# fjall-rs/lsm-tree

Measured on AMD Instinct MI355X. Metric: device-resident data-block decode+encode GiB/s, 1 M × 4 KiB blocks, higher is better.
Workload: dtype u8; 1 GPU; BASELINE configs[1]/[2]: encode + decode round trip of 1 M x 4 KiB data blocks, device-resident; blocks_per_gpu=1048576, items_per_gpu=54525952, block_bytes_per_gpu=3953267212, restart_interval=16, key_len=16, val_len=64, parallelism=shard1 (independent block batches, no collective)

## Files before the change

### lsm-tree_amd/csrc/encode.hip

```cpp
#include <hip/hip_runtime.h>

#include <math.h>

#include <algorithm>
#include <cstddef>
#include <type_traits>

#include "block_format.hpp"
#include "decode.hpp"
#include "encode.hpp"
#include "scan.hpp"
#include "fill.hpp"

namespace lsmgpu {

constexpr uint32_t kPlanHuge = 1, kPlanBad = 2, kPlanMedium = 4, kPlanBig = 8;
constexpr uint32_t kPlanHugeGpu = 16;
constexpr uint32_t kImgMedium = 20 * 1024;
constexpr uint32_t kImgBig = 96 * 1024;
constexpr uint32_t kListBigWaves = 8;
constexpr uint32_t kE3HashChunk = 4096;
constexpr uint64_t kListedOne = 1ULL << 40, kOffMask = kListedOne - 1;

struct alignas(16) BlockPlan {
// ... 1058 lines not shown
      for (uint32_t q = 0; q < kPW; ++q) {
        if (!ok[q]) continue;
        const uint32_t n = bst[jq[q] + 1] - bst[jq[q]];
        const uint32_t buckets = bucket_count(n, P.ratio);
        const uint32_t hw = (buckets > 0 && (n + ri - 1) / ri <= kHashMaxPointers) ? buckets : 0;
        uint32_t hb = kNoBucket;
        if (hw && hw < kNeedHash) {
          if (m[q].klen <= 16)
            hb = (uint32_t)(xxh3_64_le16(m[q].klen, WinReader8{wb[q].lo, wb[q].hi},
                                         WinReader64{wb[q].lo, wb[q].hi}) % hw);
          else
            hb = kNeedHash, P.hb_fix[0] = 1;
        }
        P.hbucket[(uint64_t)base + t0 + q] = (uint16_t)hb;
      }
    }
    wave_lds_sync();
    uint32_t nq[kPW];
    uint64_t hq[kPW];
#pragma unroll
    for (uint32_t q = 0; q < kPW; ++q) {
      nq[q] = 0;
      hq[q] = 0;
      wa[q] = wb[q];
      if (ok[q] && jjq[q] % ri != 0) {
        const uint32_t h = base + t0 + q - jjq[q] % ri;
        const bool in = h >= base;
        const uint64_t hko = in ? (uint64_t)wkos[h - base] : hk_ko;
        const uint32_t hkl = in ? wkls[h - base] : hk_kl;
        nq[q] = min(hkl, m[q].klen);
        hq[q] = hko;
        wa[q] = in ? wkwin[h - base] : hk_win;
      }
    }
#pragma unroll
    for (uint32_t q = 0; q < kPW; ++q) {
      if (!nq[q]) continue;
      const uint64_t x0 = wa[q].lo ^ wb[q].lo, x1 = wa[q].hi ^ wb[q].hi;
      const uint32_t n = nq[q];
      uint32_t sh;
      if (x0) sh = min(n, (uint32_t)(__builtin_ctzll(x0) >> 3));
      else if (x1) sh = min(n, 8 + (uint32_t)(__builtin_ctzll(x1) >> 3));
      else sh = n <= 16 ? n : lcp_tail(P.it.keys, hq[q], m[q].ko, n);
      m[q].sh = sh;
    }
    uint64_t rec[kPW], tsum = 0;
#pragma unroll
    for (uint32_t q = 0; q < kPW; ++q) {
      rec[q] = ok[q] ? item_record_len(P, m[q], jjq[q] % ri == 0) : 0;
      tsum += rec[q];
    }
    const uint64_t incl = wave_incl_scan_u64(tsum);
    uint64_t ex = carry + incl - tsum;
    uint64_t exq[kPW];
#pragma unroll
    for (uint32_t q = 0; q < kPW; ++q) {
      exq[q] = ex;
      if (ok[q]) {
        const uint32_t jb = jq[q], jj = jjq[q], ridx = jj / ri;
        const uint32_t n = bst[jb + 1] - bst[jb];
        if (jj == 0) bfirst[jb] = ex;
        if (jj + 1 == n) bend[jb] = ex + rec[q];
        if (jj == ridx * ri && ridx == (n - 1) / ri) lhead[jb] = ex;
      }
      ex += rec[q];
    }
    wave_lds_sync();
#pragma unroll
    for (uint32_t q = 0; q < kPW; ++q) {
      if (ok[q]) {
        const uint32_t jj = jjq[q], ridx = jj / ri;
        const bool head = jj == ridx * ri;
        const uint64_t roff = exq[q] - bfirst[jq[q]];
        const uint32_t x = head ? ridx : m[q].sh;
        P.erec[(uint64_t)base + t0 + q] =
            bst[jq[q] + 1] - bst[jq[q]] > kGItems
                ? (uint32_t)min(roff, (uint64_t)0xFFFFFFFFu)
                : (uint32_t)min(roff, (uint64_t)0x7FFF) | (head ? kErecHead : 0u) | (min(x, 0xFFFFu) << 16);
      }
    }
    carry += wave_bcast_u64(incl, kWave - 1);
    {
      const uint32_t last = min(ie, base + kPWStep) - 1, ll = (last - base) / kPW, lq = (last - base) % kPW;
      uint32_t jsel = jjq[0];
#pragma unroll
      for (uint32_t q = 1; q < kPW; ++q) jsel = lq == q ? jjq[q] : jsel;
      const uint32_t jjl = __builtin_amdgcn_readlane((int)jsel, (int)ll);
      const uint32_t h = last - jjl % ri;
      if (h >= base) {
        hk_ko = wkos[h - base];
        hk_kl = wkls[h - base];
        hk_win = wkwin[h - base];
      }
    }
    wave_lds_sync();
  }
  __syncthreads();
  if (tid >= nb) return;
  const uint32_t b = b0 + tid, s = bst[tid], e = bst[tid + 1];
  bool bad = !mono || e <= s || badf[tid] || start_past_items(P, b + 1);
  const uint32_t n = bad ? 0 : e - s;
  const uint64_t recs = bad ? 0 : bend[tid] - bfirst[tid], last_head = bad ? 0 : lhead[tid] - bfirst[tid];
  const uint32_t bin_len = n ? (n + ri - 1) / ri : 0;
  const uint32_t step = last_head <= 0xFFFF ? 2 : 4;
  const uint32_t buckets = bucket_count(n, P.ratio);
  const uint32_t hash_w = (buckets > 0 && bin_len <= kHashMaxPointers) ? buckets : 0;
  const uint64_t total = kHdrLen + recs + 1 + (uint64_t)bin_len * step + hash_w + kTrailerLen;
  if (recs > 0xFFFFFFF0ULL || total > 0xFFFFFF00ULL) bad = true;
  const uint64_t ks = koff<kOW>(P, s), ke = koff<kOW>(P, e);
  const uint64_t vs = voff<kOW>(P, s), ve = voff<kOW>(P, e);
  uint32_t flags = 0;
  if (bad) {
    flags = kPlanBad;
    P.status[b] = ST_BAD_ARG;
  } else if (!group_fits(n, ke - ks, ve - vs, total, hash_w)) {
    const uint64_t need = e2_need(total, hash_w);
    flags = need <= kImgMedium ? kPlanMedium : need <= kImgBig ? kPlanBig : kPlanHuge;
  }
  const BlockPlan pl{(uint32_t)recs, bin_len, hash_w, step | (flags << 8)};
  const uint64_t size = (bad ? 0 : total) | ((flags & (kPlanMedium | kPlanBig | kPlanHuge)) ? kListedOne : 0);
  P.plans[b] = pl;
  if (kFused) {
    fplan[tid] = pl;
    fsize[tid] = size;
    if (size & ~kOffMask) P.status[b] = ST_INCOMPLETE;
  } else {
    P.sizes[b] = size;
  }
  P.kspan[b] = ks;
  P.vspan[b] = vs;
  if (b + 1 == P.n_blocks) {
    P.kspan[b + 1] = ke;
    P.vspan[b + 1] = ve;
  }
}

template <bool kBkt, int kOW>
__global__ __launch_bounds__(256) __attribute__((amdgpu_waves_per_eu(4))) void encode_plan_wave_kernel(EncodeParams P) {
  __shared__ PlanWaveLds S;
  const uint32_t b0 = blockIdx.x * P.plan_bpw;
  plan_wave_run<kBkt, kOW, false>(P, b0, min(P.plan_bpw, P.n_blocks - b0), S, nullptr, nullptr);
}

struct GBlk {
  uint32_t it0, n;
  uint32_t img, plen;
  uint32_t recs, bin_len;
  uint32_t step, hash_w;
  uint32_t hash_base, u0;
  uint32_t nbk, spare;
};
static_assert(sizeof(GBlk) == 48, "GBlk");

struct GroupLds {
  uint8_t keys[kGKeys + kGSlack];
  uint8_t vals[kGVals + kGSlack];
  uint8_t img[kGImg + kGSlack];
  uint32_t uni[kGUnion / 4];
  GBlk blk[2][kGBlocks];
  LongSecret secret;
};
static_assert(offsetof(GroupLds, uni) - offsetof(GroupLds, vals) >= sizeof(PlanWaveLds), "plan LDS over the stage");
static_assert(offsetof(GroupLds, vals) % 16 == 0, "plan LDS alignment");
static_assert(kGRunFused * (sizeof(BlockPlan) + 8) + 16 <= kGUnion, "fused plan outputs in uni");


__device__ __forceinline__ void lds_copy(uint8_t* dst, uint32_t d, const uint8_t* src, uint32_t s, uint32_t n,
                                         uint32_t rot, uint32_t done = 0) {
  if (!n) return;
  const uint32_t h = min(n, (4u - (d & 3u)) & 3u);
  uint32_t hb[3];
#pragma unroll
  for (uint32_t k = 0; k < 3; ++k)
    if (k < h) hb[k] = src[s + k];
#pragma unroll
  for (uint32_t k = 0; k < 3; ++k)
    if (k < h) dst[d + k] = (uint8_t)hb[k];
  if (n == h) return;
  const uint32_t d1 = d + h + 4 * done, e = d + n, body = ((e & ~3u) - d1) >> 2;
  const uint32_t sp = s + h + 4 * done, sh = sp & 3u;
  const uint32_t* s32 = reinterpret_cast<const uint32_t*>(src + (sp & ~3u));
  uint32_t* d32 = reinterpret_cast<uint32_t*>(dst + d1);
  uint32_t q = ((rot & 31u) * body) >> 5;
  constexpr uint32_t U = 4;
  const uint32_t w0 = body ? s32[0] : 0;
  uint32_t carry = body ? s32[q] : 0;
  for (uint32_t j0 = 0; j0 < body; j0 += U) {
    uint32_t hi[U], at[U];
#pragma unroll
    for (uint32_t t = 0; t < U; ++t) {
      uint32_t p = q + t;
      p = p >= body ? p - body : p;
      at[t] = p;
      if (j0 + t < body) hi[t] = s32[p + 1];
    }
#pragma unroll
    for (uint32_t t = 0; t < U; ++t) {
      if (j0 + t < body) {
        const uint32_t lo = t == 0 ? carry : (at[t] == 0 ? w0 : hi[t - 1]);
        d32[at[t]] = alignbyte(hi[t], lo, sh);
      }
    }
    q += U;
    q = q >= body ? q - body : q;
    carry = q == 0 ? w0 : hi[U - 1];
  }
  const uint32_t t0 = d1 + 4 * body;
  uint32_t tb[3];
#pragma unroll
  for (uint32_t k = 0; k < 3; ++k)
    if (t0 + k < e) tb[k] = src[s + (t0 + k - d)];
#pragma unroll
  for (uint32_t k = 0; k < 3; ++k)
    if (t0 + k < e) dst[t0 + k] = (uint8_t)tb[k];
}

#ifdef LSM_NO_UNIFORM_COPY
constexpr bool kUniformCopy = false;
#else
constexpr bool kUniformCopy = true;
#endif
constexpr uint32_t kUniformMin = 4;
__device__ __forceinline__ uint32_t lds_copy_uniform(uint8_t* dst, uint32_t d, const uint8_t* src, uint32_t s,
                                                     uint32_t n, bool has, uint32_t rot) {
  if (!kUniformCopy) return 0;
  const uint32_t h = min(n, (4u - (d & 3u)) & 3u);
  const uint32_t body = n > h ? (((d + n) & ~3u) - (d + h)) >> 2 : 0u;
  const uint32_t B = wave_min_u32(has ? body : 0xFFFFFFFFu);
  if (B < kUniformMin || B == 0xFFFFFFFFu) return 0;
  if (has) {
    const uint8_t* sb = src + ((s + h) & ~3u);
    uint8_t* db = dst + d + h;
    const uint32_t sh = (s + h) & 3u, B4 = 4 * B;
    auto ld = [&](uint32_t x) { return *reinterpret_cast<const uint32_t*>(sb + x); };
    auto st = [&](uint32_t x, uint32_t v) { *reinterpret_cast<uint32_t*>(db + x) = v; };
    constexpr uint32_t U = kUniformMin;
    uint32_t x = (((rot & 31u) * B) >> 5) * 4;
    const uint32_t w0 = ld(0);
    uint32_t carry = ld(x);
    for (uint32_t j = 0; j < B; j += U) {
      uint32_t at[U], hi[U];
#pragma unroll
      for (uint32_t t = 0; t < U; ++t) {
        const uint32_t y = x + 4 * t;
        at[t] = t == 0 ? x : min(y, y - B4);
        hi[t] = ld(at[t] + 4);
      }
#pragma unroll
      for (uint32_t t = 0; t < U; ++t) {
        const uint32_t lo = at[t] == 0 ? w0 : (t == 0 ? carry : hi[t - 1]);
        st(at[t], alignbyte(hi[t], lo, sh));
      }
      carry = hi[U - 1];
      x += 4 * U;
      x = min(x, x - B4);
    }
    if (body > B) {
      st(B4, alignbyte(ld(B4 + 4), ld(B4), sh));
      return B + 1;
    }
  }
  return B;
}

__device__ __forceinline__ uint32_t lds_put_leb(uint8_t* dst, uint32_t pos, uint64_t v) {
  while (v >= 0x80) {
    dst[pos++] = (uint8_t)(v | 0x80);
    v >>= 7;
  }
  dst[pos++] = (uint8_t)v;
  return pos;
}

__device__ __forceinline__ void group_barrier() {
  __builtin_amdgcn_fence(__ATOMIC_RELEASE, "workgroup", "local");
  __builtin_amdgcn_s_barrier();
  __builtin_amdgcn_fence(__ATOMIC_ACQUIRE, "workgroup", "local");
}

__device__ __forceinline__ void group_barrier_lds() {
  asm volatile("s_waitcnt lgkmcnt(0)\n\ts_barrier" ::: "memory");
}

#ifdef LSM_DIAG
#define ENC_PHASE(i)                                 \
  if (P.diag & 0x80) {                              \
    const uint64_t t_ = __builtin_amdgcn_s_memtime(); \
    ph_acc[i] += (uint32_t)(t_ - t_last);            \
    t_last = t_;                                     \
  }
#else
#define ENC_PHASE(i)
#endif

__device__ __forceinline__ uint32_t block_of_item(const EncodeParams& P, uint32_t i) {
  uint32_t lo = 0, hi = P.n_blocks;
  while (hi - lo > 1) {
    const uint32_t mid = (lo + hi) >> 1;
    if (clamped_start(P, mid) <= i) lo = mid;
    else hi = mid;
  }
  return lo;
}

constexpr uint64_t kE1pBad = 1ULL << 63;
constexpr uint32_t kE1pMaxBpw = 4;
__device__ __forceinline__ uint64_t e1p_add(uint64_t a, uint64_t b) {
  return ((a | b) & kE1pBad) | ((a + b) & ~kE1pBad);
}

__device__ __forceinline__ uint64_t shfl_down64(uint64_t v, int o) {
  return (uint64_t)(uint32_t)__shfl_down((int)(uint32_t)v, o) |
         ((uint64_t)(uint32_t)__shfl_down((int)(uint32_t)(v >> 32), o) << 32);
}

constexpr uint32_t kE1pPer = 4;
constexpr uint32_t kE1pLenPer = 1;

__device__ __forceinline__ uint32_t wg_first_block(const EncodeParams& P, uint32_t first) {
  const uint32_t i_end = clamped_start(P, P.n_blocks);
  uint32_t lo = 0, hi = P.n_blocks;
  if (first >= i_end) hi = 1;
  while (hi - lo > 1) {
    const uint32_t st = (hi - lo + 255) / 256;
    const uint32_t x = lo + threadIdx.x * st;
    const uint32_t c = (uint32_t)__syncthreads_count(x < hi && clamped_start(P, x) <= first);
    const uint32_t nlo = lo + (c ? c - 1 : 0) * st;
    hi = min(hi, nlo + st);
    lo = nlo;
  }
  return lo;
}

template <uint32_t K>
struct E1pItems {
  uint32_t i[K], b[K], s[K], e[K];
  bool in[K];
};
template <uint32_t K>
__device__ __forceinline__ E1pItems<K> e1p_items(const EncodeParams& P) {
  E1pItems<K> t;
  const uint32_t i_begin = clamped_start(P, 0), i_end = clamped_start(P, P.n_blocks);
  const uint32_t base = blockIdx.x * (256 * K);
  uint32_t b = wg_first_block(P, max(base, i_begin));
  uint32_t bs = clamped_start(P, b), be = clamped_start(P, b + 1);
#pragma unroll
  for (uint32_t j = 0; j < K; ++j) {
    const uint32_t i = base + 256 * j + threadIdx.x;
    const bool in = i >= i_begin && i < i_end && (uint64_t)i < P.it.n_items;
    while (in && b + 1 < P.n_blocks && be <= i) {
      ++b;
      bs = be;
      be = clamped_start(P, b + 1);
    }
    t.i[j] = i;
    t.b[j] = b;
    t.s[j] = bs;
    t.e[j] = be;
    t.in[j] = in;
  }
  return t;
}

constexpr uint32_t kEncHugeCountWord = 2;

template <int kOW>
__global__ __launch_bounds__(256) void encode_e1p_lengths_kernel(EncodeParams P) {
  if (blockIdx.x == 0) {
    int bad = 0;
    for (uint32_t x = threadIdx.x; x < P.n_blocks; x += 256)
      bad |= clamped_start(P, x + 1) < clamped_start(P, x) ? 1 : 0;
    bad = __syncthreads_or(bad);
    if (threadIdx.x == 0) {
      P.e1p_flag[0] = bad ? 1u : 0u;
      if (P.huge_pool) reinterpret_cast<uint32_t*>(P.huge_pool)[kEncHugeCountWord] = 0;
    }
  }
  const E1pItems<kE1pLenPer> T = e1p_items<kE1pLenPer>(P);
  const uint32_t ri = P.ri, lane = threadIdx.x & 63;
  bool live[kE1pLenPer], head[kE1pLenPer];
  RawItemT<kOW> r[kE1pLenPer];
  uint64_t hko[kE1pLenPer], hko1[kE1pLenPer];
#pragma unroll
  for (uint32_t j = 0; j < kE1pLenPer; ++j) {
    const uint32_t i = T.i[j];
    live[j] = T.in[j] && T.s[j] <= i && i < T.e[j];
    head[j] = (i - T.s[j]) % ri == 0;
    hko[j] = hko1[j] = 0;
    if (live[j]) {
      r[j] = load_raw<false, kOW>(P, i);
      if (!head[j]) {
        const uint64_t h = (uint64_t)i - (i - T.s[j]) % ri;
        hko[j] = koff<kOW>(P, h);
        hko1[j] = koff<kOW>(P, h + 1);
      }
    }
  }
  ItemMeta m[kE1pLenPer];
  bool bad[kE1pLenPer];
  Win16 wa[kE1pLenPer], wb[kE1pLenPer];
#pragma unroll
  for (uint32_t j = 0; j < kE1pLenPer; ++j) {
    bad[j] = false;
    if (live[j]) {
      m[j] = cook_item<false>(r[j], bad[j]);
      if (!head[j]) {
        wa[j] = gwin16(P.it.keys + hko[j]);
        wb[j] = gwin16(P.it.keys + m[j].ko);
      }
    }
  }
#pragma unroll
  for (uint32_t j = 0; j < kE1pLenPer; ++j) {
    const uint32_t i = T.i[j];
    uint64_t rec = 0;
    if (live[j]) {
      if (!head[j]) {
        const uint32_t n = min((uint32_t)min(hko1[j] - hko[j], (uint64_t)0xFFFF), m[j].klen);
        const uint64_t x0 = wa[j].lo ^ wb[j].lo, x1 = wa[j].hi ^ wb[j].hi;
        uint32_t sh;
        if (x0) sh = min(n, (uint32_t)(__builtin_ctzll(x0) >> 3));
        else if (x1) sh = min(n, 8 + (uint32_t)(__builtin_ctzll(x1) >> 3));
        else sh = n <= 16 ? n : lcp_tail(P.it.keys, hko[j], m[j].ko, n);
        m[j].sh = sh;
// ... 206 lines not shown
    BlockPlan* const fplan = reinterpret_cast<BlockPlan*>(L.uni);
    uint64_t* const fsize = reinterpret_cast<uint64_t*>(L.uni) + 2 * kRun;
    uint64_t* const fbase = fsize + kRun;
    plan_wave_run<false, kOW, true>(P, b_begin, b_end - b_begin, *reinterpret_cast<PlanWaveLds*>(L.vals), fplan,
                                    fsize);
    __syncthreads();
    r_plan = rb < b_end ? fplan[lane] : BlockPlan{0, 0, 0, 0};
    const uint64_t sz = rb < b_end ? fsize[lane] : 0;
    const uint64_t incl = wave_incl_scan_u64(sz);
    if (wave == 0) {
      bool poisoned;
      const uint64_t base = run_lookback(P.sizes, blockIdx.x, wave_bcast_u64(incl, kWave - 1), P.diag, poisoned);
      if (lane == 0) {
        fbase[0] = base;
        fbase[1] = poisoned ? 1 : 0;
      }
    }
    __syncthreads();
    const uint64_t ex = fbase[0] + incl - sz;
    run_ok = fbase[1] == 0;
    r_off = in_run ? (ex & kOffMask) : 0;
    if (wave == 0 && rb < b_end) {
      P.block_off[rb] = r_off;
      if (!run_ok) P.status[rb] = ST_INCOMPLETE;
      else if (sz & ~kOffMask) P.lists[ex >> 40] = rb;
    }
    if (wave == 0 && rb == b_end && b_end == P.n_blocks) {
      P.block_off[rb] = r_off;
      P.list_count[0] = run_ok ? (uint32_t)(ex >> 40) : 0u;
    }
    const uint32_t cs = in_run ? clamped_start(P, rb) : 0;
    r_ks = in_run ? koff<kOW>(P, cs) : 0;
    r_vs = in_run ? voff<kOW>(P, cs) : 0;
    __syncthreads();
  } else {
    r_off = in_run ? P.block_off[rb] : 0;
    r_ks = in_run ? P.kspan[rb] : 0;
    r_vs = in_run ? P.vspan[rb] : 0;
    r_plan = (in_run && rb < b_end) ? P.plans[rb] : BlockPlan{0, 0, 0, 0};
  }
  const uint32_t r_hash = r_plan.hash_w;
  const uint32_t r_hpre = wave_incl_scan_u32(r_hash) - r_hash;
  uint32_t r_upre;
  {
    const uint64_t nx = wave_shfl_u64(r_off, min(lane + 1, 63));
    const uint32_t plen = (rb < b_end) ? (uint32_t)(nx - r_off) - kHdrLen : 0;
    const uint32_t units = plen > 240 ? (plen - 1) / 1024 + 1 : 0;
    r_upre = wave_incl_scan_u32(units) - units;
  }
  auto lane_u32 = [&](uint32_t v, uint32_t l) { return (uint32_t)__shfl((int)v, (int)min(l, 63u)); };
  auto lane_u64 = [&](uint64_t v, uint32_t l) { return wave_shfl_u64(v, (int)min(l, 63u)); };
  auto rl32 = [&](uint32_t v, uint32_t l) { return (uint32_t)__builtin_amdgcn_readlane((int)v, (int)min(l, 63u)); };
  auto rl64 = [&](uint64_t v, uint32_t l) {
    const int q = (int)min(l, 63u);
    return (uint64_t)(uint32_t)__builtin_amdgcn_readlane((int)(uint32_t)v, q) |
           ((uint64_t)(uint32_t)__builtin_amdgcn_readlane((int)(uint32_t)(v >> 32), q) << 32);
  };
  struct Grp {
    uint32_t b, k;
  };
  auto form = [&](uint32_t b) -> Grp {
    const uint32_t r0 = b - b_begin, rj = r0 + lane;
    const uint32_t s0 = rl32(r_start, r0), s1 = lane_u32(r_start, rj + 1);
    const uint64_t o0 = rl64(r_off, r0), o1 = lane_u64(r_off, rj + 1);
    const uint64_t k0 = rl64(r_ks, r0), k1 = lane_u64(r_ks, rj + 1);
    const uint64_t v0 = rl64(r_vs, r0), v1 = lane_u64(r_vs, rj + 1);
    const uint32_t flags = lane_u32(r_plan.step_flags, rj) >> 8;
    const uint32_t hsum = lane_u32(r_hpre, rj + 1) - rl32(r_hpre, r0);
    const bool ok = b + lane < b_end && lane < (int)kGBlocks && flags == 0 && o1 <= P.out_cap &&
                    group_fits(s1 - s0, k1 - (k0 & ~15ULL), v1 - (v0 & ~15ULL), o1 - (o0 & ~15ULL), hsum);
    return Grp{b, (uint32_t)__builtin_ctzll(~__ballot(ok))};
  };
  const uint64_t gmask = __ballot(rb < b_end && (r_plan.step_flags >> 8) == 0);
  auto next_group = [&](uint32_t b) -> Grp {
    for (;;) {
      if (b >= b_end) return Grp{b, 0};
      const Grp g = form(b);
      if (g.k) return g;
      const uint64_t rest = gmask >> (b - b_begin);
      if (rest & 1) {
        if (lane == 0) P.status[b] = ST_OVERFLOW;
        ++b;
      } else {
        b = rest ? b + (uint32_t)__builtin_ctzll(rest) : b_end;
      }
    }
  };
  auto issue_dma = [&](const Grp& g) {
    const uint32_t r0 = g.b - b_begin;
    const uint64_t ka = rl64(r_ks, r0) & ~15ULL, kb = rl64(r_ks, r0 + g.k);
    const uint64_t va = rl64(r_vs, r0) & ~15ULL, vb = rl64(r_vs, r0 + g.k);
    const uint32_t kc = (uint32_t)((kb - ka + 15) >> 4), vc = index ? 0 : (uint32_t)((vb - va + 15) >> 4);
    const uint8_t* ks = P.it.keys + ka + 16 * lane;
    for (uint32_t i = wave; i * kWave < kc; i += kGWaves)
      if (i * kWave + lane < kc)
        __builtin_amdgcn_global_load_lds((gbl_void_t*)(ks + 1024 * i), (lds_void_t*)(L.keys + 1024 * i), 16, 0, 0);
    const uint8_t* vs = P.it.vals + va + 16 * lane;
    for (uint32_t i = wave; i * kWave < vc; i += kGWaves)
      if (i * kWave + lane < vc)
        __builtin_amdgcn_global_load_lds((gbl_void_t*)(vs + 1024 * i), (lds_void_t*)(L.vals + 1024 * i), 16, 0, 0);
  };
  uint32_t* hlo = L.uni;
  uint32_t* hhi = hlo + kGHash;
  uint64_t* contrib = reinterpret_cast<uint64_t*>(L.uni);

  auto tpi_shift = [&](uint32_t n) -> uint32_t { return n <= kGThreads / 4 ? 2u : n <= kGThreads / 2 ? 1u : 0u; };
  auto load_items = [&](const Grp& g, RawItemT<kOW, kIndex>& r) {
    const uint32_t r0 = g.b - b_begin;
    const uint32_t i0 = rl32(r_start, r0), n = rl32(r_start, r0 + g.k) - i0;
    const uint64_t i = (uint64_t)i0 + min(tid >> tpi_shift(n), n - 1);
    r = load_raw<kIndex, kOW>(P, i);
    r.e = P.erec[i];
    if (kPlanBkt) r.hb = P.hbucket[i];
  };
  auto cook = [&](const RawItemT<kOW, kIndex>& r) {
    bool bad = false;
    return cook_item<kIndex>(r, bad);
  };

  auto build_table = [&](const Grp& g, GBlk* tb) {
    const uint32_t gr0 = g.b - b_begin, gk = g.k;
    const uint32_t gi0 = rl32(r_start, gr0);
    const uint64_t gob = rl64(r_off, gr0);
    const uint32_t gpad = (uint32_t)(((uint64_t)(uintptr_t)P.out + gob) & 15);
    const uint32_t rj = gr0 + lane;
    const uint32_t st = lane_u32(r_start, rj), st1 = lane_u32(r_start, rj + 1);
    const uint64_t of = lane_u64(r_off, rj), of1 = lane_u64(r_off, rj + 1);
    const uint32_t recs = lane_u32(r_plan.recs, rj), bin_len = lane_u32(r_plan.bin_len, rj);
    const uint32_t sf = lane_u32(r_plan.step_flags, rj), hw = lane_u32(r_plan.hash_w, rj);
    const uint32_t hb = lane_u32(r_hpre, rj) - rl32(r_hpre, gr0);
    const bool in = (uint32_t)lane < gk;
    const uint32_t plen = in ? (uint32_t)(of1 - of) - kHdrLen : 0;
    const uint32_t nbk = plen > 240 ? (plen - 1) / 1024 : 0;
    const uint32_t units = plen > 240 ? nbk + 1 : 0;
    const uint32_t u0 = wave_incl_scan_u32(units) - units;
    if (in) {
      GBlk B;
      B.it0 = st - gi0;
      B.n = st1 - st;
      B.img = (uint32_t)(of - gob) + gpad;
      B.plen = plen;
      B.recs = recs;
      B.bin_len = bin_len;
      B.step = sf & 0xFF;
      B.hash_w = hw;
      B.hash_base = hb;
      B.u0 = u0;
      B.nbk = nbk;
      B.spare = 0;
      tb[lane] = B;
    }
  };

#ifdef LSM_DIAG
  uint64_t t_last = __builtin_amdgcn_s_memtime();
  uint32_t ph_acc[12] = {};
  uint32_t ph_n = 0;
#endif
  Grp G = run_ok ? next_group(b_begin) : Grp{b_end, 0};
  RawItemT<kOW, kIndex> raw{};
  if (G.k) {
    issue_dma(G);
    load_items(G, raw);
    if (wave == 0) build_table(G, L.blk[0]);
  }
  __builtin_amdgcn_s_waitcnt(0x0070);
  ENC_PHASE(11);
  uint32_t iter = 0;
  while (G.k) {
    ENC_PHASE(0);
    const uint32_t r0 = G.b - b_begin, k = G.k;
    const uint32_t i0 = rl32(r_start, r0), n_items = rl32(r_start, r0 + k) - i0;
    const uint64_t kbase = rl64(r_ks, r0) & ~15ULL, vbase = rl64(r_vs, r0) & ~15ULL;
    const uint64_t obase = rl64(r_off, r0);
    const uint64_t dabs = (uint64_t)(uintptr_t)P.out + obase;
    const uint32_t pad = (uint32_t)(dabs & 15);
    const uint32_t tsh = tpi_shift(n_items), part = tid & ((1u << tsh) - 1), item = tid >> tsh;
    const bool live = item < n_items;
    const Grp Gn = next_group(G.b + k);
    ItemMeta m = cook(raw);
    if (Gn.k) load_items(Gn, raw);
    ENC_PHASE(9);
    GBlk* const TB = L.blk[iter & 1];
    const uint32_t hsum = rl32(r_hpre, r0 + k) - rl32(r_hpre, r0);
    for (uint32_t h = tid; h < hsum; h += kGThreads) {
      hlo[h] = 0xFFFFFFFFu;
      hhi[h] = 0;
    }
    group_barrier_lds();
    ENC_PHASE(1);
    uint32_t j = 0;
    for (uint32_t jb = 1; jb < k; ++jb) j += (rl32(r_start, r0 + jb) - i0 <= item) ? 1u : 0u;
    const bool head = (m.e & kErecHead) != 0;
    m.sh = head ? 0u : m.e >> 16;
    const bool writes = live && !(kDiagBuild && (P.diag & 9));
    const uint32_t roff = m.e & 0x7FFFu;
    const uint32_t from = head ? 0 : m.sh;
    const uint32_t kst = (uint32_t)(m.ko - kbase);
    const bool has_val = writes && !index && !is_tombstone(m.vt);
    const uint32_t vsrc = (uint32_t)(m.vo - vbase);
    auto put_header = [&]() -> uint32_t {
      uint32_t pos = TB[j].img + kHdrLen + roff;
      if (index) {
        L.img[pos++] = 0;
        pos = lds_put_leb(L.img, pos, m.vo);
        pos = lds_put_leb(L.img, pos, m.vl);
        pos = lds_put_leb(L.img, pos, m.seq);
        pos = lds_put_leb(L.img, pos, m.klen);
        lds_copy(L.img, pos, L.keys, kst, m.klen, lane);
      } else {
        L.img[pos++] = (uint8_t)m.vt;
        pos = lds_put_leb(L.img, pos, m.seq);
        if (!head) pos = lds_put_leb(L.img, pos, m.sh);
        pos = lds_put_leb(L.img, pos, m.klen - from);
        lds_copy(L.img, pos, L.keys, kst + from, m.klen - from, lane);
        pos += m.klen - from;
        if (!is_tombstone(m.vt)) pos = lds_put_leb(L.img, pos, m.vl);
      }
      return pos;
    };
    auto put_index_and_vote = [&]() {
      const GBlk& B = TB[j];
      if (head) {
        const uint32_t bp = B.img + kHdrLen + B.recs + 1 + (m.e >> 16) * B.step;
        for (uint32_t q = 0; q < B.step; ++q) L.img[bp + q] = (uint8_t)(roff >> (8 * q));
      }
      if (kHash && B.hash_w) {
        const uint32_t ridx = (item - B.it0) / ri;
        const uint32_t hb =
            kPlanBkt ? m.hb
                     : (uint32_t)(xxh3_64_any(m.klen, BaseReader8{L.keys, kst}, BaseReader64{L.keys, kst}) % B.hash_w);
        const uint32_t bk = B.hash_base + hb;
        atomicMin(&hlo[bk], ridx);
        atomicMax(&hhi[bk], ridx);
      }
    };
    constexpr bool uniform = !index;
    if (tsh == 0) {
      uint32_t vpos = 0;
      if (writes) vpos = put_header();
      const uint32_t done =
          uniform ? lds_copy_uniform(L.img, vpos, L.vals, vsrc, m.vl, has_val && m.vl != 0, lane) : 0u;
      if (writes) {
        if (has_val) lds_copy(L.img, vpos, L.vals, vsrc, m.vl, lane, done);
        put_index_and_vote();
      }
    } else {
      const uint32_t va = (part * m.vl) >> tsh, vb = ((part + 1) * m.vl) >> tsh;
      uint32_t vpos = 0;
      if (writes) {
        if (part == 0)
          vpos = put_header();
        else if (has_val)
          vpos = TB[j].img + kHdrLen + roff + 1 + leb_len(m.seq) + (head ? 0u : leb_len(m.sh)) + leb_len(m.klen - from) +
                 (m.klen - from) + leb_len(m.vl);
      }
      const uint32_t done =
          uniform ? lds_copy_uniform(L.img, vpos + va, L.vals, vsrc + va, vb - va, has_val && vb != va, lane) : 0u;
      if (writes) {
        if (has_val) lds_copy(L.img, vpos + va, L.vals, vsrc + va, vb - va, lane, done);
        if (part == 0) put_index_and_vote();
      }
    }
    auto tails = [&]() {
      for (uint32_t jb = wave; jb < (kDiagBuild && (P.diag & 8) ? 0 : k); jb += kGWaves) {
        const GBlk& B = TB[jb];
        const uint32_t p0 = B.img + kHdrLen, bin_off = B.recs + 1;
        if (lane == 0) L.img[p0 + B.recs] = kTrailerMarker;
        const uint32_t hash_off = B.hash_w ? bin_off + B.bin_len * B.step : 0;
        if (kHash)
          for (uint32_t q = lane; q < B.hash_w; q += kWave)
            L.img[p0 + hash_off + q] = (uint8_t)bucket_byte(hlo[B.hash_base + q], hhi[B.hash_base + q]);
        write_trailer_bytes(L.img, p0 + B.plen - kTrailerLen, ri, B.step, B.bin_len, bin_off, B.hash_w, hash_off,
                            B.n);
      }
    };
    if (!kHash) tails();
    group_barrier_lds();
    ENC_PHASE(3);
    if (Gn.k && !(kDiagBuild && (P.diag & 16))) issue_dma(Gn);
    ENC_PHASE(10);
    if (kHash) {
      tails();
      group_barrier_lds();
    }
    ENC_PHASE(4);
    {
      const uint32_t row = wave * 4 + (lane >> 4), r = lane & 15, q = r & 3, s = r >> 2;
      const uint32_t ubase = rl32(r_upre, r0);
      const uint32_t units = (kDiagBuild && (P.diag & 10)) ? 0 : rl32(r_upre, r0 + k) - ubase;
      const uint64_t* acc = L.secret.acc + s + 2 * q;
      for (uint32_t u = row; u < units; u += 4 * kGWaves) {
        uint32_t jb = 0;
        for (uint32_t x = 1; x < k; ++x) jb += (rl32(r_upre, r0 + x) - ubase <= u) ? 1u : 0u;
        const GBlk& B = TB[jb];
        const uint32_t n = u - B.u0, p0 = B.img + kHdrLen;
        uint64_t c0 = 0, c1 = 0;
        if (n < B.nbk) {
#pragma unroll
          for (int t = 0; t < 4; ++t) {
            const Win16 w = read_win16(L.img, p0 + n * 1024 + 256 * t + 16 * r);
            stripe_part(w, acc[4 * t], acc[4 * t + 1], c0, c1);
          }
        } else {
          const uint32_t tail0 = B.nbk * 1024, nb_stripes = ((B.plen - 1) - tail0) / 64;
#pragma unroll
          for (int t = 0; t < 4; ++t) {
            if ((uint32_t)(4 * t + s) < nb_stripes) {
              const Win16 w = read_win16(L.img, p0 + tail0 + 256 * t + 16 * r);
              stripe_part(w, acc[4 * t], acc[4 * t + 1], c0, c1);
            }
          }
          if (r < 4) {
            const Win16 w = read_win16(L.img, p0 + B.plen - 64 + 16 * r);
            stripe_part(w, L.secret.last[2 * q], L.secret.last[2 * q + 1], c0, c1);
          }
        }
        c0 = row_quad_sum64(c0);
        c1 = row_quad_sum64(c1);
        if (r < 4) {
          contrib[8 * u + 2 * q] = c0;
          contrib[8 * u + 2 * q + 1] = c1;
        }
      }
    }
    group_barrier_lds();
    ENC_PHASE(5);
    const uint32_t cw = iter & (kGWaves - 1);
    const uint32_t total = (uint32_t)(rl64(r_off, r0 + k) - obase);
    const uint32_t end = (kDiagBuild && (P.diag & 4)) ? pad : pad + total;
    const uint32_t c0 = (pad + 15) >> 4, c1 = end >> 4;
    const u32x4* const csrc = reinterpret_cast<const u32x4*>(L.img);
    u32x4* const cdst = reinterpret_cast<u32x4*>(dabs & ~15ULL);
    const uint32_t hpc = (wave == cw && (uint32_t)lane < 3 * k) ? (TB[lane / 3].img >> 4) + lane % 3 : ~0u;
    if (wave == cw) {
      if (!(kDiagBuild && (P.diag & 10))) {
        const uint32_t jb = (uint32_t)lane >> 2;
        const int q = lane & 3;
        const bool in = jb < k;
        const GBlk& B = TB[in ? jb : 0];
        const uint32_t p0 = B.img + kHdrLen, plen = B.plen;
        uint64_t lo = 0, hi = 0;
        if (in && plen > 240) {
          uint64_t a0 = q == 0 ? (uint64_t)P32_3 : q == 1 ? P64_2 : q == 2 ? P64_4 : P64_5;
          uint64_t a1 = q == 0 ? P64_1 : q == 1 ? P64_3 : q == 2 ? (uint64_t)P32_2 : (uint64_t)P32_1;
          const uint64_t scr0 = L.secret.acc[16 + 2 * q], scr1 = L.secret.acc[16 + 2 * q + 1];
          const uint64_t* cb = contrib + 8 * B.u0 + 2 * q;
          for (uint32_t n0 = 0; n0 < B.nbk; n0 += 4) {
            uint64_t c0[4], c1[4];
#pragma unroll
            for (uint32_t t = 0; t < 4; ++t) {
              c0[t] = cb[8 * (n0 + t)];
              c1[t] = cb[8 * (n0 + t) + 1];
            }
#pragma unroll
            for (uint32_t t = 0; t < 4; ++t) {
              if (n0 + t < B.nbk) {
                a0 = xxh3_scr(a0, c0[t], scr0);
                a1 = xxh3_scr(a1, c1[t], scr1);
              }
            }
          }
          a0 += cb[8 * B.nbk];
          a1 += cb[8 * B.nbk + 1];
          lo = mul_fold64(a0 ^ L.secret.mlo[2 * q], a1 ^ L.secret.mlo[2 * q + 1]);
          hi = mul_fold64(a0 ^ L.secret.mhi[2 * q], a1 ^ L.secret.mhi[2 * q + 1]);
        }
        lo = quad_sum64(lo);
        hi = quad_sum64(hi);
        if (in) {
          if (plen > 240) {
            lo = xxh3_avalanche((uint64_t)plen * P64_1 + lo);
            hi = xxh3_avalanche(~((uint64_t)plen * P64_2) + hi);
          } else {
            xxh3_128_short(plen, BaseReader8{L.img, p0}, BaseReader64{L.img, p0}, lo, hi);
          }
          write_header_quad(L.img, B.img, P.type, lo, hi, plen, q);
          if (q == 0) P.status[G.b + jb] = ST_OK;
        }
// ... 810 lines not shown
```

Measured before the change: 927.7 GiB/s.

## Add per-wave block encode loop with private LDS slots for small blocks

Adds a fast path in the group encode kernel where each wave independently encodes whole blocks into its own LDS slot when every block in the range fits. The slot is fed by direct global-to-LDS DMA, with the next block prefetched, then the block is hashed and copied out. This drops the workgroup-wide barriers, the group table build and the cross-wave coordination for the common small-block case. It also factors the header and bin-entry writers into shared helpers, and it pads the LDS struct, which risks lower occupancy if the size grows.

Measured after the change: 982.6 GiB/s, median of 6. 5.9% higher.

```diff
diff --git a/lsm-tree_amd/csrc/encode.hip b/lsm-tree_amd/csrc/encode.hip
--- a/lsm-tree_amd/csrc/encode.hip
+++ b/lsm-tree_amd/csrc/encode.hip
@@ -1234,17 +1234,48 @@
 };
 static_assert(sizeof(GBlk) == 48, "GBlk");
 
+#ifdef LSM_NO_WAVE_BLOCKS
+constexpr bool kWaveBlocks = false;
+#else
+constexpr bool kWaveBlocks = true;
+#endif
+constexpr uint32_t kWKeys = 1024, kWVals = 4096, kWImg = 4496;
+constexpr uint32_t kWItems = kWave;
+constexpr uint32_t kWUnits = 5;
+static_assert((kWImg - 1) / 1024 <= 4 && (kWImg - 1) / 1024 + 1 <= kWUnits,
+              "full KiB units and the tail unit of a payload");
+constexpr uint32_t kDiagNoWaveBlocks = 0x20;
+struct WaveSlot {
+  uint8_t keys[kWKeys + kGSlack];
+  uint8_t vals[kWVals + kGSlack];
+  uint8_t img[kWImg + kGSlack];
+  uint64_t contrib[kWUnits * 8];
+};
+static_assert(offsetof(WaveSlot, vals) % 16 == 0 && offsetof(WaveSlot, img) % 16 == 0 && sizeof(WaveSlot) % 16 == 0,
+              "stage DMA and 16-B copy-out alignment");
+constexpr uint32_t kGroupBody = kGKeys + kGVals + kGImg + 3 * kGSlack + kGUnion + 2 * kGBlocks * (uint32_t)sizeof(GBlk);
+constexpr uint32_t kWaveSlots = kGWaves * (uint32_t)sizeof(WaveSlot);
+constexpr uint32_t kWavePad = kWaveSlots > kGroupBody ? kWaveSlots - kGroupBody : 16;
+
 struct GroupLds {
   uint8_t keys[kGKeys + kGSlack];
   uint8_t vals[kGVals + kGSlack];
   uint8_t img[kGImg + kGSlack];
   uint32_t uni[kGUnion / 4];
   GBlk blk[2][kGBlocks];
+  uint8_t wave_pad[kWavePad];
   LongSecret secret;
 };
 static_assert(offsetof(GroupLds, uni) - offsetof(GroupLds, vals) >= sizeof(PlanWaveLds), "plan LDS over the stage");
 static_assert(offsetof(GroupLds, vals) % 16 == 0, "plan LDS alignment");
 static_assert(kGRunFused * (sizeof(BlockPlan) + 8) + 16 <= kGUnion, "fused plan outputs in uni");
+static_assert(offsetof(GroupLds, wave_pad) == kGroupBody, "GroupLds layout");
+static_assert(kGWaves * sizeof(WaveSlot) <= offsetof(GroupLds, secret), "the wave slots lie over the group loop's LDS");
+static_assert(sizeof(GroupLds) <= 40960, "four workgroups per CU");
+
+__device__ __host__ __forceinline__ bool wave_fits(uint64_t n, uint64_t kspan, uint64_t vspan, uint64_t total) {
+  return n >= 1 && n <= kWItems && kspan + 15 <= kWKeys && vspan + 15 <= kWVals && total + 15 <= kWImg;
+}
 
 
 __device__ __forceinline__ void lds_copy(uint8_t* dst, uint32_t d, const uint8_t* src, uint32_t s, uint32_t n,
@@ -1352,6 +1383,32 @@
   }
   dst[pos++] = (uint8_t)v;
   return pos;
+}
+
+template <bool kIndex>
+__device__ __forceinline__ uint32_t put_record_header(uint8_t* img, uint32_t pos, const uint8_t* keys, uint32_t kst,
+                                                      const ItemMeta& m, bool head, uint32_t from, uint32_t rot) {
+  if (kIndex) {
+    img[pos++] = 0;
+    pos = lds_put_leb(img, pos, m.vo);
+    pos = lds_put_leb(img, pos, m.vl);
+    pos = lds_put_leb(img, pos, m.seq);
+    pos = lds_put_leb(img, pos, m.klen);
+    lds_copy(img, pos, keys, kst, m.klen, rot);
+  } else {
+    img[pos++] = (uint8_t)m.vt;
+    pos = lds_put_leb(img, pos, m.seq);
+    if (!head) pos = lds_put_leb(img, pos, m.sh);
+    pos = lds_put_leb(img, pos, m.klen - from);
+    lds_copy(img, pos, keys, kst + from, m.klen - from, rot);
+    pos += m.klen - from;
+    if (!is_tombstone(m.vt)) pos = lds_put_leb(img, pos, m.vl);
+  }
+  return pos;
+}
+
+__device__ __forceinline__ void put_bin_entry(uint8_t* img, uint32_t bp, const uint32_t& step, uint32_t roff) {
+  for (uint32_t q = 0; q < step; ++q) img[bp + q] = (uint8_t)(roff >> (8 * q));
 }
 
 __device__ __forceinline__ void group_barrier() {
@@ -1864,6 +1921,172 @@
     }
   };
 
+  constexpr bool kWaveLoop = kWaveBlocks && !kIndex && !kHash && !kPlanBkt && !kFused;
+  if constexpr (kWaveLoop) {
+    bool wave_run;
+    {
+      const uint32_t s1 = lane_u32(r_start, lane + 1);
+      const uint64_t o1 = lane_u64(r_off, lane + 1), k1 = lane_u64(r_ks, lane + 1), v1 = lane_u64(r_vs, lane + 1);
+      const bool fit = (r_plan.step_flags >> 8) == 0 && o1 <= P.out_cap &&
+                       wave_fits(s1 - r_start, k1 - (r_ks & ~15ULL), v1 - (r_vs & ~15ULL), o1 - (r_off & ~15ULL));
+      wave_run = __ballot(rb < b_end && !fit) == 0 && !(kDiagBuild && (P.diag & (kDiagNoWaveBlocks | 0x9F)));
+    }
+    if (wave_run) {
+      WaveSlot& W = reinterpret_cast<WaveSlot*>(&L)[wave];
+      auto wave_lds_wait = [&]() { asm volatile("s_waitcnt lgkmcnt(0)" ::: "memory"); };
+      auto wave_dma = [&](uint32_t r) {
+        const uint64_t ka = rl64(r_ks, r) & ~15ULL, kb = rl64(r_ks, r + 1);
+        const uint64_t va = rl64(r_vs, r) & ~15ULL, vb = rl64(r_vs, r + 1);
+        const uint32_t kc = (uint32_t)((kb - ka + 15) >> 4), vc = (uint32_t)((vb - va + 15) >> 4);
+        const uint8_t* ks = P.it.keys + ka + 16 * lane;
+        for (uint32_t i = 0; i * kWave < kc; ++i)
+          if (i * kWave + lane < kc)
+            __builtin_amdgcn_global_load_lds((gbl_void_t*)(ks + 1024 * i), (lds_void_t*)(W.keys + 1024 * i), 16, 0, 0);
+        const uint8_t* vs = P.it.vals + va + 16 * lane;
+        for (uint32_t i = 0; i * kWave < vc; ++i)
+          if (i * kWave + lane < vc)
+            __builtin_amdgcn_global_load_lds((gbl_void_t*)(vs + 1024 * i), (lds_void_t*)(W.vals + 1024 * i), 16, 0, 0);
+      };
+      auto wave_items = [&](uint32_t r, RawItemT<kOW, kIndex>& x) {
+        const uint32_t i0 = rl32(r_start, r), n = rl32(r_start, r + 1) - i0;
+        const uint64_t i = (uint64_t)i0 + min((uint32_t)lane, n - 1);
+        x = load_raw<kIndex, kOW>(P, i);
+        x.e = P.erec[i];
+      };
+      group_barrier_lds();
+      uint32_t r = wave;
+      const uint32_t nr = b_end - b_begin;
+      RawItemT<kOW, kIndex> raw{};
+      if (r < nr) {
+        wave_dma(r);
+        wave_items(r, raw);
+      }
+      asm volatile("s_waitcnt vmcnt(0)" ::: "memory");
+      while (r < nr) {
+        const uint32_t i0 = rl32(r_start, r), n = rl32(r_start, r + 1) - i0;
+        const uint64_t kbase = rl64(r_ks, r) & ~15ULL, vbase = rl64(r_vs, r) & ~15ULL;
+        const uint64_t obase = rl64(r_off, r);
+        const uint32_t total = (uint32_t)(rl64(r_off, r + 1) - obase), plen = total - kHdrLen;
+        const uint32_t recs = rl32(r_plan.recs, r), bin_len = rl32(r_plan.bin_len, r);
+        const uint32_t step = rl32(r_plan.step_flags, r) & 0xFF;
+        const uint64_t dabs = (uint64_t)(uintptr_t)P.out + obase;
+        const uint32_t pad = (uint32_t)(dabs & 15), p0 = pad + kHdrLen;
+        const uint32_t rn = r + kGWaves;
+        const bool more = rn < nr;
+        ItemMeta m = cook(raw);
+        if (more) wave_items(rn, raw);
+        {
+          const bool live = (uint32_t)lane < n;
+          const bool head = (m.e & kErecHead) != 0;
+          m.sh = head ? 0u : m.e >> 16;
+          const uint32_t roff = m.e & 0x7FFFu, from = head ? 0 : m.sh;
+          const uint32_t kst = (uint32_t)(m.ko - kbase), vsrc = (uint32_t)(m.vo - vbase);
+          const bool has_val = live && !is_tombstone(m.vt);
+          uint32_t vpos = 0;
+          if (live) vpos = put_record_header<false>(W.img, p0 + roff, W.keys, kst, m, head, from, lane);
+          const uint32_t done = lds_copy_uniform(W.img, vpos, W.vals, vsrc, m.vl, has_val && m.vl != 0, lane);
+          if (live) {
+            if (has_val) lds_copy(W.img, vpos, W.vals, vsrc, m.vl, lane, done);
+            if (head) put_bin_entry(W.img, p0 + recs + 1 + (m.e >> 16) * step, step, roff);
+          }
+        }
+        if (lane == 0) W.img[p0 + recs] = kTrailerMarker;
+        write_trailer_bytes(W.img, p0 + plen - kTrailerLen, ri, step, bin_len, recs + 1, 0, 0, n);
+        wave_lds_wait();
+        if (more) wave_dma(rn);
+        uint64_t lo = 0, hi = 0;
+        const int q = lane & 3;
+        if (plen > 240) {
+          const uint32_t nbk = (plen - 1) / 1024;
+          {
+            const uint32_t row = (uint32_t)lane >> 4, rr = lane & 15, s = rr >> 2;
+            const uint64_t* acc = L.secret.acc + s + 2 * q;
+            for (uint32_t u = row; u <= nbk; u += 4) {
+              uint64_t c0 = 0, c1 = 0;
+              if (u < nbk) {
+#pragma unroll
+                for (int t = 0; t < 4; ++t) {
+                  const Win16 w = read_win16(W.img, p0 + u * 1024 + 256 * t + 16 * rr);
+                  stripe_part(w, acc[4 * t], acc[4 * t + 1], c0, c1);
+                }
+              } else {
+                const uint32_t tail0 = nbk * 1024, nb_stripes = ((plen - 1) - tail0) / 64;
+#pragma unroll
+                for (int t = 0; t < 4; ++t) {
+                  if ((uint32_t)(4 * t + s) < nb_stripes) {
+                    const Win16 w = read_win16(W.img, p0 + tail0 + 256 * t + 16 * rr);
+                    stripe_part(w, acc[4 * t], acc[4 * t + 1], c0, c1);
+                  }
+                }
+                if (rr < 4) {
+                  const Win16 w = read_win16(W.img, p0 + plen - 64 + 16 * rr);
+                  stripe_part(w, L.secret.last[2 * q], L.secret.last[2 * q + 1], c0, c1);
+                }
+              }
+              c0 = row_quad_sum64(c0);
+              c1 = row_quad_sum64(c1);
+              if (rr < 4) {
+                W.contrib[8 * u + 2 * q] = c0;
+                W.contrib[8 * u + 2 * q + 1] = c1;
+              }
+            }
+          }
+          wave_lds_wait();
+          uint64_t a0 = q == 0 ? (uint64_t)P32_3 : q == 1 ? P64_2 : q == 2 ? P64_4 : P64_5;
+          uint64_t a1 = q == 0 ? P64_1 : q == 1 ? P64_3 : q == 2 ? (uint64_t)P32_2 : (uint64_t)P32_1;
+          const uint64_t scr0 = L.secret.acc[16 + 2 * q], scr1 = L.secret.acc[16 + 2 * q + 1];
+          const uint64_t* cb = W.contrib + 2 * q;
+          uint64_t c0[4], c1[4];
+#pragma unroll
+          for (uint32_t t = 0; t < 4; ++t) {
+            c0[t] = cb[8 * t];
+            c1[t] = cb[8 * t + 1];
+          }
+          const uint64_t t0 = cb[8 * nbk], t1 = cb[8 * nbk + 1];
+#pragma unroll
+          for (uint32_t t = 0; t < 4; ++t) {
+            if (t < nbk) {
+              a0 = xxh3_scr(a0, c0[t], scr0);
+              a1 = xxh3_scr(a1, c1[t], scr1);
+            }
+          }
+          a0 += t0;
+          a1 += t1;
+          lo = mul_fold64(a0 ^ L.secret.mlo[2 * q], a1 ^ L.secret.mlo[2 * q + 1]);
+          hi = mul_fold64(a0 ^ L.secret.mhi[2 * q], a1 ^ L.secret.mhi[2 * q + 1]);
+        }
+        lo = quad_sum64(lo);
+        hi = quad_sum64(hi);
+        if (lane < 4) {
+          if (plen > 240) {
+            lo = xxh3_avalanche((uint64_t)plen * P64_1 + lo);
+            hi = xxh3_avalanche(~((uint64_t)plen * P64_2) + hi);
+          } else {
+            xxh3_128_short(plen, BaseReader8{W.img, p0}, BaseReader64{W.img, p0}, lo, hi);
+          }
+          write_header_quad(W.img, pad, P.type, lo, hi, plen, q);
+          if (lane == 0) P.status[b_begin + r] = ST_OK;
+        }
+        wave_lds_wait();
+        asm volatile("s_waitcnt vmcnt(0)" ::: "memory");
+        {
+          const uint32_t end = pad + total, c0 = (pad + 15) >> 4, c1 = end >> 4;
+          const u32x4* const csrc = reinterpret_cast<const u32x4*>(W.img);
+          u32x4* const cdst = reinterpret_cast<u32x4*>(dabs & ~15ULL);
+          for (uint32_t c = c0 + (uint32_t)lane; c < c1; c += kWave)
+            *(__attribute__((address_space(1))) u32x4*)(cdst + c) = csrc[c];
+          auto* gb = (__attribute__((address_space(1))) uint8_t*)cdst;
+          const uint32_t x = (uint32_t)lane;
+          if (x >= pad && x < min(16 * c0, end)) gb[x] = W.img[x];
+          if (c1 >= c0 && 16 * c1 + x < end) gb[16 * c1 + x] = W.img[16 * c1 + x];
+        }
+        wave_lds_wait();
+        r = rn;
+      }
+      return;
+    }
+  }
+
 #ifdef LSM_DIAG
   uint64_t t_last = __builtin_amdgcn_s_memtime();
   uint32_t ph_acc[12] = {};
@@ -1912,31 +2135,11 @@
     const bool has_val = writes && !index && !is_tombstone(m.vt);
     const uint32_t vsrc = (uint32_t)(m.vo - vbase);
     auto put_header = [&]() -> uint32_t {
-      uint32_t pos = TB[j].img + kHdrLen + roff;
-      if (index) {
-        L.img[pos++] = 0;
-        pos = lds_put_leb(L.img, pos, m.vo);
-        pos = lds_put_leb(L.img, pos, m.vl);
-        pos = lds_put_leb(L.img, pos, m.seq);
-        pos = lds_put_leb(L.img, pos, m.klen);
-        lds_copy(L.img, pos, L.keys, kst, m.klen, lane);
-      } else {
-        L.img[pos++] = (uint8_t)m.vt;
-        pos = lds_put_leb(L.img, pos, m.seq);
-        if (!head) pos = lds_put_leb(L.img, pos, m.sh);
-        pos = lds_put_leb(L.img, pos, m.klen - from);
-        lds_copy(L.img, pos, L.keys, kst + from, m.klen - from, lane);
-        pos += m.klen - from;
-        if (!is_tombstone(m.vt)) pos = lds_put_leb(L.img, pos, m.vl);
-      }
-      return pos;
+      return put_record_header<index>(L.img, TB[j].img + kHdrLen + roff, L.keys, kst, m, head, from, lane);
     };
     auto put_index_and_vote = [&]() {
       const GBlk& B = TB[j];
-      if (head) {
-        const uint32_t bp = B.img + kHdrLen + B.recs + 1 + (m.e >> 16) * B.step;
-        for (uint32_t q = 0; q < B.step; ++q) L.img[bp + q] = (uint8_t)(roff >> (8 * q));
-      }
+      if (head) put_bin_entry(L.img, B.img + kHdrLen + B.recs + 1 + (m.e >> 16) * B.step, B.step, roff);
       if (kHash && B.hash_w) {
         const uint32_t ridx = (item - B.it0) / ri;
         const uint32_t hb =
```
